# KaHIP/KaMinPar

Measured on NVIDIA H100. Metric: lp_edges_per_second, higher is better.
Workload: dtype int32

## Files before the change

kaminpar_b200/csrc/lp_device.cuh:

```cuda
#pragma once

#include <cstdint>
#include <cuda_runtime.h>

namespace kmp {

constexpr uint32_t kEmpty = 0xFFFFFFFFu;
constexpr unsigned kFull = 0xFFFFFFFFu;
constexpr int kLadderLevels = 16;

enum : uint32_t { SALT_SUBROUND = 1, SALT_TIE = 2, SALT_FAV = 3, SALT_COMMIT = 4 };

__host__ __device__ __forceinline__ uint32_t lowbias32(uint32_t x) {
  x ^= x >> 16;
  x *= 0x7FEB352Du;
  x ^= x >> 15;
  x *= 0x846CA68Bu;
  x ^= x >> 16;
  return x;
}
__host__ __device__ __forceinline__ uint32_t tie_hash(uint32_t base, uint32_t u, uint32_t c) {
  return lowbias32((u * 0x9E3779B1u) ^ (c * 0x85EBCA77u) ^ base);
}
__host__ __device__ __forceinline__ uint32_t bijective32(uint32_t x, uint32_t base) {
  x ^= base;
  x *= 0x9E3779B1u;
  x ^= x >> 15;
  x *= 0x85EBCA77u;
  x ^= x >> 13;
  x *= 0xC2B2AE3Du;
  x ^= x >> 16;
  return x;
}
__host__ __device__ __forceinline__ uint32_t subround_of(uint32_t u, uint32_t granule_log2,
                                                         uint32_t base, uint32_t S) {
  const uint32_t h = lowbias32((u >> granule_log2) ^ base);
  return static_cast<uint32_t>((static_cast<uint64_t>(h) * S) >> 32);
}
__device__ __forceinline__ uint32_t ladder_level(uint32_t prio) {
  const uint32_t z = static_cast<uint32_t>(__clz(static_cast<int>(prio)));
  return z < static_cast<uint32_t>(kLadderLevels - 1) ? z : static_cast<uint32_t>(kLadderLevels - 1);
}
__host__ __device__ __forceinline__ uint32_t degree_group(uint32_t d) {
  return d < 8 ? 0u : (d < 32 ? 1u : (d < 256 ? 2u : 3u));
}

inline uint64_t splitmix64(uint64_t x) {
  x += 0x9E3779B97F4A7C15ull;
  x = (x ^ (x >> 30)) * 0xBF58476D1CE4E5B9ull;
  x = (x ^ (x >> 27)) * 0x94D049BB133111EBull;
  return x ^ (x >> 31);
}
inline uint32_t sync_base(int seed, uint32_t call, uint32_t iter, uint32_t salt) {
  const uint64_t a = splitmix64((static_cast<uint64_t>(static_cast<uint32_t>(seed)) << 32) | call);
  const uint64_t b = splitmix64((static_cast<uint64_t>(iter) << 32) | salt);
  return static_cast<uint32_t>(splitmix64(a ^ b) >> 32);
}

struct Cand {
  int32_t gain;
  int32_t over;
  uint32_t hash;
  uint32_t key;
};
__device__ __forceinline__ Cand cand_none() { return Cand{-1, 0, kEmpty, kEmpty}; }

template <int MODE> __device__ __forceinline__ bool cand_better(const Cand &a, const Cand &b) {
  if (a.gain != b.gain) {
    return a.gain > b.gain;
  }
  if (MODE == 1 && a.over != b.over) {
    return a.over < b.over;
  }
  if (a.hash != b.hash) {
    return a.hash < b.hash;
  }
  return a.key < b.key;
}

template <int MODE> __device__ __forceinline__ Cand warp_argmax(unsigned mask, Cand c) {
  const int gmax = __reduce_max_sync(mask, c.gain);
  bool in = (c.gain == gmax) && (gmax > 0);
  int omin = 0;
  if (MODE == 1) {
    omin = __reduce_min_sync(mask, in ? c.over : INT32_MAX);
    in = in && (c.over == omin);
  }
  const unsigned hmin = __reduce_min_sync(mask, in ? c.hash : kEmpty);
  in = in && (c.hash == hmin);
  const unsigned kmin = __reduce_min_sync(mask, in ? c.key : kEmpty);
  Cand r;
  r.gain = gmax > 0 ? gmax : -1;
  r.over = omin;
  r.hash = hmin;
  r.key = kmin;
  return r;
}

constexpr uint32_t kStampBits = 6;
constexpr uint32_t kMaxStampSubrounds = 1u << kStampBits;
template <bool P64> struct LabG;
template <> struct LabG<false> {
  using word = uint32_t;
  static __host__ __device__ __forceinline__ uint32_t label(word w) { return w & 0x00FFFFFFu; }
  static __host__ __device__ __forceinline__ uint32_t stamp(word w) { return w >> 24; }
  static __host__ __device__ __forceinline__ word pack(uint32_t label, uint32_t stamp) { return label | (stamp << 24); }
};
template <> struct LabG<true> {
  using word = unsigned long long;
  static __host__ __device__ __forceinline__ uint32_t label(word w) { return static_cast<uint32_t>(w); }
  static __host__ __device__ __forceinline__ uint32_t stamp(word w) { return static_cast<uint32_t>(w >> 32); }
  static __host__ __device__ __forceinline__ word pack(uint32_t label, uint32_t stamp) {
    return static_cast<word>(label) | (static_cast<word>(stamp) << 32);
  }
};
__host__ __device__ __forceinline__ uint32_t make_stamp(uint32_t round, uint32_t subround) {
  return 1u + ((round & 1u) << kStampBits) + subround;
}
struct StampWindow {
  uint32_t start, len;
};
__host__ __device__ __forceinline__ StampWindow make_window(uint32_t round, uint32_t subround) {
  return StampWindow{(((round & 1u) ^ 1u) << kStampBits) + subround, (2u << kStampBits) - subround};
}
__device__ __forceinline__ bool stamp_hit(uint32_t stamp, const StampWindow &w) {
  return stamp != 0 && ((stamp - 1u - w.start) & ((2u << kStampBits) - 1u)) < w.len;
}

constexpr int kCounterNodesOffset = 16;
struct SweepArgs {
  const uint32_t *__restrict__ xadj;
  const uint32_t *__restrict__ adjncy;
  const int32_t *__restrict__ vwgt;
  const int32_t *__restrict__ adjwgt;
  const uint32_t *__restrict__ label;
  const void *__restrict__ labg;
  StampWindow window;
  bool pull;
  uint32_t *__restrict__ queue;
  const int32_t *__restrict__ weight;
  const int32_t *__restrict__ max_w;
  const int32_t *__restrict__ min_w;
  const uint32_t *__restrict__ communities;
  uint8_t *__restrict__ active;
  uint32_t *__restrict__ favored;
  int32_t max_cluster_weight;
  uint32_t num_labels;
  uint32_t max_num_neighbors;
  const uint32_t *__restrict__ list;
  uint32_t list_size;
  uint32_t base_tie, base_fav, base_commit;
  uint32_t *__restrict__ mv_u;
  uint32_t *__restrict__ mv_t;
  uint32_t *__restrict__ mover_count;
  bool accumulate;
  int32_t *__restrict__ incoming;
  int32_t *__restrict__ hist;
  unsigned long long *__restrict__ counters;
  uint32_t *__restrict__ sel_target;
  uint32_t *__restrict__ sel_favored;
};

template <int MODE>
__device__ __forceinline__ Cand eval_candidate_w(const SweepArgs &a, uint32_t u, uint32_t own, int32_t uw,
                                                 int32_t own_w, uint32_t key, int32_t rating, int32_t kw,
                                                 bool store_fav, Cand &fav) {
  Cand c = cand_none();
  fav = cand_none();
  if (rating <= 0) {
    return c;
  }
  if (MODE == 0) {
    bool feasible = (kw + uw <= a.max_cluster_weight) || (key == own);
    if (a.communities != nullptr) {
      feasible = feasible && (a.communities[key] == a.communities[own]);
    }
    if (feasible) {
      c.gain = rating;
      c.over = 0;
      c.hash = tie_hash(a.base_tie, u, key);
      c.key = key;
    }
    if (store_fav) {
      fav.gain = rating;
      fav.over = 0;
      fav.hash = tie_hash(a.base_fav, u, key);
      fav.key = key;
    }
  } else {
    const int32_t kmax = a.max_w[key];
    const int32_t over = kw - kmax;
    const int32_t init_over = own_w - a.max_w[own];
    const bool feasible = (kw + uw <= kmax) || (over < init_over) || (key == own);
    if (feasible) {
      c.gain = rating;
      c.over = over;
      c.hash = tie_hash(a.base_tie, u, key);
      c.key = key;
    }
  }
  return c;
}

template <int MODE>
__device__ __forceinline__ Cand eval_candidate(const SweepArgs &a, uint32_t u, uint32_t own, int32_t uw,
                                               int32_t own_w, uint32_t key, int32_t rating, bool store_fav,
                                               Cand &fav) {
  if (rating <= 0) {
    fav = cand_none();
    return cand_none();
  }
  return eval_candidate_w<MODE>(a, u, own, uw, own_w, key, rating, a.weight[key], store_fav, fav);
}

template <int MODE>
__device__ __forceinline__ bool finish_vertex(const SweepArgs &a, uint32_t u, uint32_t own, bool store_fav,
                                              const Cand &best, const Cand &fav, uint32_t &target_out) {
  const uint32_t target = best.gain > 0 ? best.key : own;
  target_out = target;
  if (a.sel_target != nullptr) {
    a.sel_target[u] = target;
    if (MODE == 0 && a.sel_favored != nullptr) {
      a.sel_favored[u] = store_fav ? (fav.gain > 0 ? fav.key : own) : kEmpty;
    }
    return false;
  }
  if (target != own) {
    return true;
  }
  if (MODE == 0 && store_fav) {
    a.favored[u] = fav.gain > 0 ? fav.key : own;
  }
  return false;
}

}
```

kaminpar_b200/csrc/lp_sweep.cuh:

```cuda
#pragma once

#include "lp_device.cuh"
#include "lp_sortnet.cuh"

namespace kmp {

template <int MODE>
__device__ __forceinline__ void emit_proposal(const SweepArgs &a, uint32_t idx, uint32_t u, uint32_t target,
                                              int32_t uw) {
  a.mv_u[idx] = u;
  a.mv_t[idx] = target;
  if (!a.accumulate) {
    return;
  }
  if (MODE == 0) {
    atomicAdd(&a.incoming[target], uw);
  } else {
    const uint32_t lvl = ladder_level(bijective32(u, a.base_commit));
    atomicAdd(&a.hist[target * kLadderLevels + lvl], uw);
  }
}

__device__ __forceinline__ void block_count_flush(const SweepArgs &a, unsigned long long edges,
                                                  unsigned long long nodes) {
  for (int o = 16; o > 0; o >>= 1) {
    edges += __shfl_xor_sync(kFull, edges, o);
    nodes += __shfl_xor_sync(kFull, nodes, o);
  }
  if ((threadIdx.x & 31) == 0 && nodes != 0) {
    atomicAdd(&a.counters[0], edges);
    atomicAdd(&a.counters[kCounterNodesOffset], nodes);
  }
}

template <bool P64>
__device__ __forceinline__ typename LabG<P64>::word load_labg(const SweepArgs &a, uint32_t v) {
  return static_cast<const typename LabG<P64>::word *>(a.labg)[v];
}

template <int R> struct ThreadRow {
  uint32_t u, beg, deg;
  uint32_t v[R > 0 ? R : 1];
};
template <int R> __device__ __forceinline__ void load_row(const SweepArgs &a, ThreadRow<R> &r) {
  r.beg = a.xadj[r.u];
  const uint32_t deg = a.xadj[r.u + 1] - r.beg;
  r.deg = deg > a.max_num_neighbors ? a.max_num_neighbors : deg;
#pragma unroll
  for (int j = 0; j < R; ++j) {
    r.v[j] = j < static_cast<int>(r.deg) ? a.adjncy[r.beg + j] : 0u;
  }
}

template <int MODE, bool EW, bool P64, int N, int R>
__device__ __forceinline__ bool sweep_thread_vertex(const SweepArgs &a, const ThreadRow<R> &r, bool flag,
                                                    unsigned long long &edges, unsigned long long &nodes,
                                                    uint32_t &target, int32_t &uw) {
  const uint32_t u = r.u;
  const uint32_t own = a.label[u];
  uw = a.vwgt != nullptr ? a.vwgt[u] : 1;
  const int32_t own_w = a.weight[own];
  uint32_t keys[N];
  int32_t ws[N];
  bool hit = false;
#pragma unroll
  for (int j = 0; j < N; ++j) {
    keys[j] = kEmpty;
    ws[j] = 0;
    if (j < static_cast<int>(r.deg)) {
      const uint32_t v = R > 0 ? r.v[j] : a.adjncy[r.beg + j];
      const typename LabG<P64>::word g = load_labg<P64>(a, v);
      hit = hit || stamp_hit(LabG<P64>::stamp(g), a.window);
      bool ok = true;
      if (MODE == 1 && a.communities != nullptr) {
        ok = a.communities[u] == a.communities[v];
      }
      if (ok) {
        keys[j] = LabG<P64>::label(g);
        ws[j] = EW ? a.adjwgt[r.beg + j] : 1;
      }
    }
  }
  if (!(flag || hit)) {
    return false;
  }
  edges += r.deg;
  nodes += 1;
  if (a.active != nullptr && flag) {
    a.active[u] = 0;
  }
  bool skip = false;
  if (MODE == 1) {
    const int32_t mn = a.min_w != nullptr ? a.min_w[own] : 0;
    skip = (own_w - uw) < mn;
  }
  const bool store_fav = (MODE == 0) && (uw == own_w) && (own_w <= a.max_cluster_weight / 2);
  Cand best = cand_none(), fav = cand_none();
  if (!skip) {
    sort_registers<N, EW>(keys, ws);
    bool lazy_done = false;
    if (MODE == 0) {
      Cand top = cand_none();
      int32_t run = 0;
#pragma unroll
      for (int j = 0; j < N; ++j) {
        run += EW ? ws[j] : 1;
        const bool last = (j == N - 1) || (keys[j + 1 < N ? j + 1 : j] != keys[j]);
        if (last) {
          const int32_t rating = run;
          run = 0;
          if (keys[j] != kEmpty && rating > 0) {
            if (rating >= top.gain) {
              const Cand x{rating, 0, tie_hash(a.base_tie, u, keys[j]), keys[j]};
              if (cand_better<0>(x, top)) {
                top = x;
              }
            }
            if (store_fav && rating >= fav.gain) {
              const Cand y{rating, 0, tie_hash(a.base_fav, u, keys[j]), keys[j]};
              if (cand_better<0>(y, fav)) {
                fav = y;
              }
            }
          }
        }
      }
      bool top_ok = true;
      if (top.gain > 0) {
        top_ok = (a.weight[top.key] + uw <= a.max_cluster_weight) || (top.key == own);
        if (a.communities != nullptr) {
          top_ok = top_ok && (a.communities[top.key] == a.communities[own]);
        }
      }
      if (top_ok) {
        best = top;
        lazy_done = true;
      }
    }
    if (!lazy_done) {
      int32_t run = 0;
#pragma unroll
      for (int j = 0; j < N; ++j) {
        run += EW ? ws[j] : 1;
        const bool last = (j == N - 1) || (keys[j + 1 < N ? j + 1 : j] != keys[j]);
        if (last) {
          const int32_t rating = run;
          run = 0;
          if (keys[j] != kEmpty) {
            Cand f;
            const Cand c = eval_candidate<MODE>(a, u, own, uw, own_w, keys[j], rating, MODE == 0 ? false : store_fav, f);
            if (cand_better<MODE>(c, best)) {
              best = c;
            }
          }
        }
      }
    }
  }
  return finish_vertex<MODE>(a, u, own, store_fav, best, fav, target);
}

template <int MODE>
__device__ __forceinline__ void emit_cta_iteration(const SweepArgs &a, bool proposes, uint32_t u, uint32_t target,
                                                   int32_t uw, uint32_t it, uint32_t (&s_cnt)[2][8],
                                                   uint32_t (&s_base)[2]) {
  const unsigned ballot = __ballot_sync(kFull, proposes);
  const int lane = threadIdx.x & 31;
  const int wib = threadIdx.x >> 5;
  const int par = it & 1;
  if (lane == 0) {
    s_cnt[par][wib] = static_cast<uint32_t>(__popc(ballot));
  }
  __syncthreads();
  if (threadIdx.x == 0) {
    uint32_t total = 0;
    for (int w = 0; w < 8; ++w) {
      total += s_cnt[par][w];
    }
    s_base[par] = total != 0 ? atomicAdd(a.mover_count, total) : 0u;
  }
  __syncthreads();
  if (proposes) {
    uint32_t idx = s_base[par] + __popc(ballot & ((1u << lane) - 1u));
    for (int w = 0; w < wib; ++w) {
      idx += s_cnt[par][w];
    }
    emit_proposal<MODE>(a, idx, u, target, uw);
  }
}

template <int MODE, bool EW, bool P64, int N> __global__ void __launch_bounds__(256) sweep_thread(const SweepArgs a) {
  __shared__ uint32_t s_cnt[2][8];
  __shared__ uint32_t s_base[2];
  unsigned long long edges = 0, nodes = 0;
  const uint32_t stride = gridDim.x * blockDim.x;
  const uint32_t bound = (a.list_size + 255u) & ~255u;
  uint32_t it = 0;
  for (uint32_t i = blockIdx.x * blockDim.x + threadIdx.x; i < bound; i += stride, ++it) {
    bool proposes = false;
    uint32_t target = 0;
    int32_t uw = 1;
    ThreadRow<0> r;
    r.u = 0;
    if (i < a.list_size) {
      r.u = a.list[i];
      const bool flag = a.active == nullptr || a.active[r.u] != 0;
      if (flag || a.pull) {
        load_row<0>(a, r);
        proposes = sweep_thread_vertex<MODE, EW, P64, N>(a, r, flag, edges, nodes, target, uw);
      }
    }
    emit_cta_iteration<MODE>(a, proposes, r.u, target, uw, it, s_cnt, s_base);
  }
  block_count_flush(a, edges, nodes);
}

__device__ __forceinline__ uint32_t pow2_ceil(uint32_t x) {
  return x <= 1 ? 1u : (1u << (32 - __clz(static_cast<int>(x - 1))));
}

__device__ __forceinline__ void table_add(uint32_t *keys, int32_t *vals, uint32_t mask, bool direct, uint32_t key,
                                          int32_t w) {
  uint32_t slot = direct ? key : (lowbias32(key) & mask);
  while (true) {
    const uint32_t prev = atomicCAS(&keys[slot], kEmpty, key);
    if (prev == kEmpty || prev == key) {
      atomicAdd(&vals[slot], w);
      return;
    }
    slot = (slot + 1) & mask;
  }
}

template <int T> struct TeamSync {
  static __device__ __forceinline__ void sync(int id) {
    if (T == 32) {
      __syncwarp();
    } else {
      asm volatile("bar.sync %0, %1;" ::"r"(id), "r"(T) : "memory");
    }
  }
  static __device__ __forceinline__ bool any(int id, bool p) {
    if (T == 32) {
      __syncwarp();
      return __any_sync(kFull, p);
    } else {
      int r;
      asm volatile(
          "{\n"
          ".reg .pred q, r;\n"
          "setp.ne.s32 q, %3, 0;\n"
          "bar.red.or.pred r, %1, %2, q;\n"
          "selp.s32 %0, 1, 0, r;\n"
          "}\n"
          : "=r"(r)
          : "r"(id), "r"(T), "r"(static_cast<int>(p))
          : "memory");
      return r != 0;
    }
  }
};

template <int MODE, int T>
__device__ __forceinline__ Cand team_argmax(int id, int tid, Cand c, Cand *s_red) {
  Cand r = warp_argmax<MODE>(kFull, c);
  if (T == 32) {
    return r;
  }
  TeamSync<T>::sync(id);
  if ((tid & 31) == 0) {
    s_red[tid >> 5] = r;
  }
  TeamSync<T>::sync(id);
  Cand x = cand_none();
  if ((tid & 31) < T / 32) {
    x = s_red[tid & 31];
  }
  return warp_argmax<MODE>(kFull, x);
}

template <bool V16> struct TeamVals;
template <> struct TeamVals<false> {
  using word = int32_t;
  static constexpr int kBytesPerSlot = 4;
  static __device__ __forceinline__ void add(word *v, uint32_t slot, int32_t w) { atomicAdd(&v[slot], w); }
  static __device__ __forceinline__ int32_t get(const word *v, uint32_t slot) { return v[slot]; }
  static __device__ __forceinline__ void clear(word *v, uint32_t slot) { v[slot] = 0; }
};
template <> struct TeamVals<true> {
  using word = uint32_t;
  static constexpr int kBytesPerSlot = 2;
  static __device__ __forceinline__ void add(word *v, uint32_t slot, int32_t w) {
    atomicAdd(&v[slot >> 1], static_cast<uint32_t>(w) << ((slot & 1u) * 16u));
  }
  static __device__ __forceinline__ int32_t get(const word *v, uint32_t slot) {
    return static_cast<int32_t>((v[slot >> 1] >> ((slot & 1u) * 16u)) & 0xFFFFu);
  }
  static __device__ __forceinline__ void clear(word *v, uint32_t slot) { reinterpret_cast<uint16_t *>(v)[slot] = 0; }
};

template <bool V16, bool EW>
__device__ __forceinline__ bool team_table_add(uint32_t *keys, typename TeamVals<V16>::word *vals, uint32_t mask,
                                               bool direct, uint32_t key, int32_t w, uint32_t &slot) {
  slot = direct ? key : (lowbias32(key) & mask);
  while (true) {
    const uint32_t prev = atomicCAS(&keys[slot], kEmpty, key);
    if (!EW && prev == kEmpty) {
      return true;
    }
    if (prev == kEmpty || prev == key) {
      TeamVals<V16>::add(vals, slot, w);
      return prev == kEmpty;
    }
    slot = (slot + 1) & mask;
  }
}
template <bool V16, bool EW>
__device__ __forceinline__ int32_t team_rating(const typename TeamVals<V16>::word *vals, uint32_t slot) {
  return TeamVals<V16>::get(vals, slot) + (EW ? 0 : 1);
}

template <int T> constexpr int team_ctas_per_sm() { return T == 32 ? 6 : T == 1024 ? 1 : 3; }

template <int MODE, bool EW, bool P64, int T, int SLOTS, int TEAMS, bool V16 = false>
__global__ void __launch_bounds__(T *TEAMS, team_ctas_per_sm<T>()) sweep_team(const SweepArgs a) {
  static_assert((SLOTS & (SLOTS - 1)) == 0, "table size must be a power of two");
  static_assert(SLOTS <= 65536, "claim lists hold 16-bit slot indices");
  static_assert(!(V16 && EW), "16-bit ratings need unit edge weights");
  using TV = TeamVals<V16>;
  constexpr int kListCap = SLOTS / 2;
  extern __shared__ __align__(16) unsigned char smem_raw[];
  __shared__ Cand s_red_all[TEAMS][T > 32 ? T / 32 : 1];
  __shared__ uint16_t s_list_all[TEAMS][kListCap];
  __shared__ uint32_t s_next[TEAMS], s_claims[TEAMS];
  __shared__ unsigned long long s_edges[TEAMS], s_nodes[TEAMS];
  const int team = threadIdx.x / T;
  const int tid = threadIdx.x % T;
  const int lane = threadIdx.x & 31;
  const int bar = 1 + team;
  uint32_t *keys = reinterpret_cast<uint32_t *>(smem_raw) + static_cast<size_t>(team) * SLOTS;
  typename TV::word *vals = reinterpret_cast<typename TV::word *>(
      smem_raw + sizeof(uint32_t) * SLOTS * TEAMS + static_cast<size_t>(team) * SLOTS * TV::kBytesPerSlot);
  Cand *s_red = s_red_all[team];
  uint16_t *list = s_list_all[team];
  for (int s = tid; s < SLOTS; s += T) {
    keys[s] = kEmpty;
    TV::clear(vals, s);
  }
  uint32_t next = 0;
  unsigned long long edges = 0, nodes = 0;
  if (tid == 0) {
    next = atomicAdd(a.queue, 1u);
    if (T > 32) {
      s_edges[team] = 0;
      s_nodes[team] = 0;
    }
  }
  TeamSync<T>::sync(bar);
  while (true) {
    uint32_t i;
    if (T == 32) {
      i = __shfl_sync(kFull, next, 0);
    } else {
      if (tid == 0) {
        s_next[team] = next;
        s_claims[team] = 0;
      }
      TeamSync<T>::sync(bar);
      i = s_next[team];
    }
    if (i >= a.list_size) {
      break;
    }
    if (tid == 0) {
      next = atomicAdd(a.queue, 1u);
    }
    const uint32_t u = a.list[i];
    const bool flag = a.active == nullptr || a.active[u] != 0;
    if (!flag && !a.pull) {
      TeamSync<T>::sync(bar);
      continue;
    }
    const uint32_t beg = a.xadj[u];
    uint32_t deg = a.xadj[u + 1] - beg;
    if (deg > a.max_num_neighbors) {
      deg = a.max_num_neighbors;
    }
    const uint32_t own = a.label[u];
    const int32_t uw = a.vwgt != nullptr ? a.vwgt[u] : 1;
    const int32_t own_w = a.weight[own];
    bool skip = false;
    if (MODE == 1) {
      const int32_t mn = a.min_w != nullptr ? a.min_w[own] : 0;
      skip = (own_w - uw) < mn;
    }
    const bool direct = a.num_labels <= static_cast<uint32_t>(SLOTS);
    bool hit = false;
    uint32_t claims = 0;
    constexpr int B = 4;
    for (uint32_t e0 = 0; e0 < deg; e0 += T * B) {
      uint32_t kb[B];
      int32_t wb[B];
      uint32_t vb[B];
#pragma unroll
      for (int j = 0; j < B; ++j) {
        const uint32_t e = e0 + j * T + tid;
        vb[j] = e < deg ? a.adjncy[beg + e] : kEmpty;
        wb[j] = (EW && e < deg) ? a.adjwgt[beg + e] : 1;
      }
#pragma unroll
      for (int j = 0; j < B; ++j) {
        kb[j] = kEmpty;
        if (vb[j] != kEmpty) {
          const typename LabG<P64>::word g = load_labg<P64>(a, vb[j]);
          hit = hit || stamp_hit(LabG<P64>::stamp(g), a.window);
          bool ok = !skip;
          if (MODE == 1 && a.communities != nullptr) {
            ok = ok && a.communities[u] == a.communities[vb[j]];
          }
          if (ok) {
            kb[j] = LabG<P64>::label(g);
          }
        }
      }
      uint32_t sl[B];
      unsigned claimed[B];
#pragma unroll
      for (int j = 0; j < B; ++j) {
        sl[j] = 0;
        claimed[j] = __ballot_sync(kFull, kb[j] != kEmpty && team_table_add<V16, EW>(keys, vals, SLOTS - 1, direct,
                                                                                     kb[j], wb[j], sl[j]));
      }
      uint32_t n = 0;
#pragma unroll
      for (int j = 0; j < B; ++j) {
        n += __popc(claimed[j]);
      }
      if (n != 0) {
        uint32_t base = claims;
        if (T == 32) {
          claims += n;
        } else {
          if (lane == 0) {
            base = atomicAdd(&s_claims[team], n);
          }
          base = __shfl_sync(kFull, base, 0);
        }
        const unsigned below = (1u << lane) - 1u;
#pragma unroll
        for (int j = 0; j < B; ++j) {
          if ((claimed[j] >> lane) & 1u) {
            list[base + __popc(claimed[j] & below)] = static_cast<uint16_t>(sl[j]);
          }
          base += __popc(claimed[j]);
        }
      }
    }
    const bool any_hit = TeamSync<T>::any(bar, hit);
    const bool act = flag || any_hit;
    const uint32_t nc = T == 32 ? claims : s_claims[team];
    const bool store_fav = (MODE == 0) && (uw == own_w) && (own_w <= a.max_cluster_weight / 2);
    Cand best = cand_none(), fav = cand_none();
    if (act) {
      Cand c = cand_none(), f = cand_none();
      if (MODE == 0) {
        for (uint32_t l = tid; l < nc; l += T) {
          const uint32_t s = list[l];
          const uint32_t k = keys[s];
          const int32_t r = team_rating<V16, EW>(vals, s);
          if (r >= c.gain) {
            Cand x{r, 0, tie_hash(a.base_tie, u, k), k};
            if (cand_better<0>(x, c)) {
              c = x;
            }
          }
          if (store_fav && r >= f.gain) {
            Cand y{r, 0, tie_hash(a.base_fav, u, k), k};
            if (cand_better<0>(y, f)) {
              f = y;
            }
          }
        }
        const Cand top = team_argmax<0, T>(bar, tid, c, s_red);
        if (store_fav) {
          fav = team_argmax<0, T>(bar, tid, f, s_red);
        }
        bool top_ok = true;
        if (top.gain > 0) {
          top_ok = (a.weight[top.key] + uw <= a.max_cluster_weight) || (top.key == own);
          if (a.communities != nullptr) {
            top_ok = top_ok && (a.communities[top.key] == a.communities[own]);
          }
        }
        if (top_ok) {
          best = top;
        } else {
          Cand cb = cand_none();
          for (uint32_t l0 = 0; l0 < nc; l0 += T * 4) {
            uint32_t kk[4];
            int32_t rr[4], ww[4];
#pragma unroll
            for (int j = 0; j < 4; ++j) {
              const uint32_t l = l0 + j * T + tid;
              const uint32_t s = l < nc ? list[l] : 0u;
              kk[j] = l < nc ? keys[s] : kEmpty;
              rr[j] = l < nc ? team_rating<V16, EW>(vals, s) : 0;
            }
#pragma unroll
            for (int j = 0; j < 4; ++j) {
              ww[j] = kk[j] != kEmpty ? a.weight[kk[j]] : 0;
            }
#pragma unroll
            for (int j = 0; j < 4; ++j) {
              if (kk[j] != kEmpty) {
                Cand ff;
                const Cand cc = eval_candidate_w<0>(a, u, own, uw, own_w, kk[j], rr[j], ww[j], false, ff);
                if (cand_better<0>(cc, cb)) {
                  cb = cc;
                }
              }
            }
          }
          best = team_argmax<0, T>(bar, tid, cb, s_red);
        }
      } else {
        for (uint32_t l = tid; l < nc; l += T) {
          const uint32_t s = list[l];
          const uint32_t k = keys[s];
          Cand ff;
          const Cand cc = eval_candidate_w<1>(a, u, own, uw, own_w, k, team_rating<V16, EW>(vals, s), a.weight[k], false, ff);
          if (cand_better<1>(cc, c)) {
            c = cc;
          }
        }
        best = team_argmax<1, T>(bar, tid, c, s_red);
      }
    }
    for (uint32_t l = tid; l < nc; l += T) {
      const uint32_t s = list[l];
      keys[s] = kEmpty;
      TV::clear(vals, s);
    }
    if (act && tid == 0) {
      if (T == 32) {
        edges += deg;
        nodes += 1;
      } else {
        s_edges[team] += deg;
        s_nodes[team] += 1;
      }
      if (a.active != nullptr && flag) {
        a.active[u] = 0;
      }
      uint32_t target;
      if (finish_vertex<MODE>(a, u, own, store_fav, best, fav, target)) {
        const uint32_t idx = atomicAdd(a.mover_count, 1u);
        emit_proposal<MODE>(a, idx, u, target, uw);
      }
    }
    TeamSync<T>::sync(bar);
  }
  if (T > 32 && tid == 0) {
    edges = s_edges[team];
    nodes = s_nodes[team];
  }
  if (tid == 0 && nodes != 0) {
    atomicAdd(&a.counters[0], edges);
    atomicAdd(&a.counters[kCounterNodesOffset], nodes);
  }
}

constexpr int kChunkEdges = 2048;
constexpr int kSliceEdges = 256;
constexpr int kSliceTableSlots = 512;
constexpr int kChunkThreads = 256;
constexpr uint32_t kBucketCap = 512;
constexpr uint32_t kBucketTargetFill = 256;
constexpr uint32_t kSelTableSlots = 1024;
constexpr int kSelWarps = 4;

struct HubOverflow {
  uint32_t bucket;
  uint32_t key;
  int32_t rating;
  uint32_t pad;
};

struct HubArgs {
  const uint32_t *__restrict__ item_entry;
  const uint32_t *__restrict__ item_chunk;
  const uint32_t *__restrict__ item_u;
  const uint32_t *__restrict__ item_beg;
  const uint32_t *__restrict__ item_deg;
  uint32_t num_items;
  const uint32_t *__restrict__ table_off;
  unsigned long long *__restrict__ g_tab;
  uint32_t *__restrict__ cursor;
  HubOverflow *__restrict__ ovf;
  uint32_t *__restrict__ ovf_count;
  uint32_t ovf_cap;
  uint32_t bucket_cap;
  uint32_t sel_limit;
  uint32_t stage_adjncy;
  const uint32_t *__restrict__ sel_entry;
  const uint32_t *__restrict__ sel_piece;
  uint32_t num_sel_items;
  const uint32_t *__restrict__ sel_begin;
  Cand *__restrict__ part_best;
  Cand *__restrict__ part_fav;
  uint32_t rank, world;
  uint32_t *__restrict__ queue;
  uint32_t *__restrict__ hit;
};

__host__ __device__ __forceinline__ uint32_t hub_buckets(uint32_t full_degree) {
  const uint32_t need = (full_degree + kBucketTargetFill - 1) / kBucketTargetFill;
  uint32_t p = 1;
  while (p < need) {
    p <<= 1;
  }
  return p;
}

__device__ __forceinline__ uint32_t smem_u32(const void *p) {
  return static_cast<uint32_t>(__cvta_generic_to_shared(p));
}
__device__ __forceinline__ void mbar_init(uint64_t *bar, uint32_t count) {
  asm volatile("mbarrier.init.shared::cta.b64 [%0], %1;" ::"r"(smem_u32(bar)), "r"(count) : "memory");
}
__device__ __forceinline__ void mbar_arrive_expect_tx(uint64_t *bar, uint32_t bytes) {
  asm volatile("mbarrier.arrive.expect_tx.shared::cta.b64 _, [%0], %1;" ::"r"(smem_u32(bar)), "r"(bytes) : "memory");
}
__device__ __forceinline__ void mbar_wait(uint64_t *bar, uint32_t parity) {
  asm volatile(
      "{\n"
      ".reg .pred p;\n"
      "WAIT_LOOP:\n"
      "mbarrier.try_wait.parity.shared::cta.b64 p, [%0], %1;\n"
      "@p bra DONE;\n"
      "bra WAIT_LOOP;\n"
      "DONE:\n"
      "}\n" ::"r"(smem_u32(bar)),
      "r"(parity)
      : "memory");
}
__device__ __forceinline__ void tma_load_1d(void *dst_smem, const void *src_gmem, uint32_t bytes, uint64_t *bar) {
  asm volatile("cp.async.bulk.shared::cluster.global.mbarrier::complete_tx::bytes [%0], [%1], %2, [%3];" ::"r"(
                   smem_u32(dst_smem)),
               "l"(src_gmem), "r"(bytes), "r"(smem_u32(bar))
               : "memory");
}

struct HubItem {
  uint32_t valid;
  uint32_t u;
  uint32_t entry;
  uint32_t full_deg;
  uint32_t gbeg, gend;
  uint32_t a0;
  uint32_t staged;
};

__device__ __forceinline__ void mbar_arrive(uint64_t *bar) {
  asm volatile("mbarrier.arrive.shared::cta.b64 _, [%0];" ::"r"(smem_u32(bar)) : "memory");
}

constexpr int kHubStages = 2;
constexpr int kHubConsumerWarps = kChunkThreads / 32;
constexpr int kHubThreads = kChunkThreads + 32;
constexpr int kHubScatterSmem = kHubConsumerWarps * kSliceTableSlots * 8;

template <int MODE, bool EW, bool P64>
__global__ void __launch_bounds__(kHubThreads, 4) sweep_hub_scatter(const SweepArgs a, const HubArgs hb, uint32_t m_total) {
  extern __shared__ __align__(16) unsigned char smem_raw[];
  constexpr int kAllSlots = kHubConsumerWarps * kSliceTableSlots;
  uint32_t *all_keys = reinterpret_cast<uint32_t *>(smem_raw);
  int32_t *all_vals = reinterpret_cast<int32_t *>(smem_raw + sizeof(uint32_t) * kAllSlots);
  __shared__ __align__(16) uint32_t s_adj[kHubStages][kChunkEdges + 8];
  __shared__ __align__(8) uint64_t s_full[kHubStages];
  __shared__ __align__(8) uint64_t s_empty[kHubStages];
  __shared__ HubItem s_item[kHubStages];
  const int lane = threadIdx.x & 31;
  const int wib = threadIdx.x >> 5;
  if (threadIdx.x == 0) {
    for (int s = 0; s < kHubStages; ++s) {
      mbar_init(&s_full[s], 1);
      mbar_init(&s_empty[s], kHubConsumerWarps);
    }
    asm volatile("fence.mbarrier_init.release.cluster;" ::: "memory");
  }
  for (int s = threadIdx.x; s < kAllSlots; s += kHubThreads) {
    all_keys[s] = kEmpty;
    all_vals[s] = 0;
  }
  __syncthreads();

  if (wib == kHubConsumerWarps) {
    if (lane == 0) {
      for (uint32_t k = 0;; ++k) {
        const int stage = static_cast<int>(k % kHubStages);
        const uint32_t round = k / kHubStages;
        mbar_wait(&s_empty[stage], (round & 1u) ^ 1u);
        const uint32_t it = atomicAdd(hb.queue, 1u);
        HubItem d{};
        d.valid = 0;
        if (it >= hb.num_items) {
          d.valid = 2;
          s_item[stage] = d;
          mbar_arrive(&s_full[stage]);
          break;
        }
        const uint32_t entry = hb.item_entry[it];
        const uint32_t u = hb.item_u[it];
        const uint32_t beg0 = hb.item_beg[it];
        const uint32_t full_deg = hb.item_deg[it];
        const uint32_t chunk = hb.item_chunk[it];
        if (entry % hb.world == hb.rank && (a.active == nullptr || a.pull || a.active[u] != 0)) {
          uint32_t deg = full_deg;
          if (deg > a.max_num_neighbors) {
            deg = a.max_num_neighbors;
          }
          const uint32_t cbeg = chunk * kChunkEdges;
          bool ok = cbeg < deg;
          if (ok && MODE == 1) {
            const uint32_t own = a.label[u];
            const int32_t uw = a.vwgt != nullptr ? a.vwgt[u] : 1;
            const int32_t mn = a.min_w != nullptr ? a.min_w[own] : 0;
            ok = !((a.weight[own] - uw) < mn);
          }
          if (ok) {
            const uint32_t cend = (cbeg + kChunkEdges < deg) ? cbeg + kChunkEdges : deg;
            d.valid = 1;
            d.u = u;
            d.entry = entry;
            d.full_deg = full_deg;
            d.gbeg = beg0 + cbeg;
            d.gend = beg0 + cend;
            d.a0 = d.gbeg & ~3u;
            d.staged = 0;
            if (hb.stage_adjncy) {
              uint32_t a1 = (d.gend + 3u) & ~3u;
              const uint32_t m4 = m_total & ~3u;
              if (a1 > m4) {
                a1 = m4;
              }
              d.staged = a1 > d.a0 ? a1 - d.a0 : 0;
            }
          }
        }
        s_item[stage] = d;
        if (d.valid && d.staged > 0) {
          asm volatile("fence.proxy.async.shared::cta;" ::: "memory");
          mbar_arrive_expect_tx(&s_full[stage], d.staged * 4);
          tma_load_1d(&s_adj[stage][0], a.adjncy + d.a0, d.staged * 4, &s_full[stage]);
        } else {
          mbar_arrive(&s_full[stage]);
        }
      }
    }
    return;
  }

  uint32_t *keys = all_keys + wib * kSliceTableSlots;
  int32_t *vals = all_vals + wib * kSliceTableSlots;
  for (uint32_t k = 0;; ++k) {
    const int stage = static_cast<int>(k % kHubStages);
    const uint32_t round = k / kHubStages;
    mbar_wait(&s_full[stage], round & 1u);
    const HubItem d = s_item[stage];
    if (d.valid == 2) {
      break;
    }
    const uint32_t wbeg = d.gbeg + wib * kSliceEdges;
    const bool mine = d.valid && wbeg < d.gend;
    if (mine) {
      const uint32_t wend = wbeg + kSliceEdges < d.gend ? wbeg + kSliceEdges : d.gend;
      const uint32_t staged_end = d.a0 + d.staged;
      bool hit = false;
      for (uint32_t e0 = wbeg; e0 < wend; e0 += 128) {
        uint32_t k4[4];
        int32_t w4[4];
#pragma unroll
        for (int j = 0; j < 4; ++j) {
          const uint32_t e = e0 + j * 32 + lane;
          k4[j] = kEmpty;
          w4[j] = 0;
          if (e < wend) {
            const uint32_t v = e < staged_end ? s_adj[stage][e - d.a0] : a.adjncy[e];
            bool ok = true;
            if (MODE == 1 && a.communities != nullptr) {
              ok = a.communities[d.u] == a.communities[v];
            }
            const typename LabG<P64>::word g = load_labg<P64>(a, v);
            hit = hit || stamp_hit(LabG<P64>::stamp(g), a.window);
            if (ok) {
              k4[j] = LabG<P64>::label(g);
              w4[j] = EW ? a.adjwgt[e] : 1;
            }
          }
        }
#pragma unroll
        for (int j = 0; j < 4; ++j) {
          if (k4[j] != kEmpty) {
            table_add(keys, vals, kSliceTableSlots - 1, false, k4[j], w4[j]);
          }
        }
      }
      if (a.pull && __any_sync(kFull, hit) && lane == 0) {
        atomicOr(&hb.hit[d.entry], 1u);
      }
    }
    __syncwarp();
    if (lane == 0) {
      mbar_arrive(&s_empty[stage]);
    }
    if (mine) {
      const uint32_t pmask = hub_buckets(d.full_deg) - 1;
      const uint32_t bucket0 = hb.table_off[d.entry];
      constexpr int B = 4;
      for (uint32_t s0 = lane; s0 < kSliceTableSlots; s0 += 32 * B) {
        uint32_t kk[B], bb[B], pos[B];
        int32_t rr[B];
#pragma unroll
        for (int j = 0; j < B; ++j) {
          const uint32_t s = s0 + j * 32;
          kk[j] = keys[s];
          rr[j] = vals[s];
          if (kk[j] != kEmpty) {
            keys[s] = kEmpty;
            vals[s] = 0;
          }
        }
#pragma unroll
        for (int j = 0; j < B; ++j) {
          bb[j] = bucket0 + (lowbias32(kk[j]) & pmask);
          pos[j] = kk[j] != kEmpty ? atomicAdd(&hb.cursor[bb[j]], 1u) : 0u;
        }
#pragma unroll
        for (int j = 0; j < B; ++j) {
          if (kk[j] != kEmpty) {
            if (pos[j] < hb.bucket_cap) {
              hb.g_tab[static_cast<size_t>(bb[j]) * kBucketCap + pos[j]] =
                  (static_cast<unsigned long long>(kk[j]) << 32) | static_cast<uint32_t>(rr[j]);
            } else {
              const uint32_t o = atomicAdd(hb.ovf_count, 1u);
              if (o < hb.ovf_cap) {
                hb.ovf[o] = HubOverflow{bb[j], kk[j], rr[j], 0u};
              }
            }
          }
        }
      }
      __syncwarp();
    }
  }
}

template <int MODE> __global__ void __launch_bounds__(kSelWarps * 32) sweep_hub_select(const SweepArgs a, const HubArgs hb) {
  __shared__ uint32_t s_keys[kSelWarps][kSelTableSlots];
  __shared__ int32_t s_vals[kSelWarps][kSelTableSlots];
  __shared__ uint32_t s_claims_all[kSelWarps];
  const int lane = threadIdx.x & 31;
  const int wib = threadIdx.x >> 5;
  uint32_t *keys = s_keys[wib];
  int32_t *vals = s_vals[wib];
  uint32_t *s_claims = &s_claims_all[wib];
  for (uint32_t s = lane; s < kSelTableSlots; s += 32) {
    keys[s] = kEmpty;
    vals[s] = 0;
  }
  if (lane == 0) {
// ... 246 lines not shown
```

Baseline: 41.13 billion.

## Split warp into half-warps to process two low-degree vertices concurrently

The warp-per-vertex sweep path now grabs two vertices per queue fetch. When both have small degree, each half-warp rates one vertex, using its own half of the shared hash table and a new half-warp argmax reduction. Otherwise the two vertices are processed one after the other by the full warp. Edge and node counters are kept in spare lanes' registers instead of separate accumulators. The aim is to cut idle lanes on low-degree vertices, at the cost of halved table capacity per vertex, extra reduction passes, and more complex control flow.

```diff
diff --git a/kaminpar_b200/csrc/lp_device.cuh b/kaminpar_b200/csrc/lp_device.cuh
--- a/kaminpar_b200/csrc/lp_device.cuh
+++ b/kaminpar_b200/csrc/lp_device.cuh
@@ -89,6 +89,36 @@
   const unsigned hmin = __reduce_min_sync(mask, in ? c.hash : kEmpty);
   in = in && (c.hash == hmin);
   const unsigned kmin = __reduce_min_sync(mask, in ? c.key : kEmpty);
+  Cand r;
+  r.gain = gmax > 0 ? gmax : -1;
+  r.over = omin;
+  r.hash = hmin;
+  r.key = kmin;
+  return r;
+}
+
+template <int MODE> __device__ __forceinline__ Cand half_warp_argmax(Cand c) {
+  const bool hi = (threadIdx.x & 16u) != 0;
+  const auto max2 = [hi](int v) {
+    const int lo_r = __reduce_max_sync(kFull, hi ? INT32_MIN : v);
+    const int hi_r = __reduce_max_sync(kFull, hi ? v : INT32_MIN);
+    return hi ? hi_r : lo_r;
+  };
+  const auto min2 = [hi](auto v, decltype(v) neutral) {
+    const auto lo_r = __reduce_min_sync(kFull, hi ? neutral : v);
+    const auto hi_r = __reduce_min_sync(kFull, hi ? v : neutral);
+    return hi ? hi_r : lo_r;
+  };
+  const int gmax = max2(c.gain);
+  bool in = (c.gain == gmax) && (gmax > 0);
+  int omin = 0;
+  if (MODE == 1) {
+    omin = min2(in ? c.over : INT32_MAX, INT32_MAX);
+    in = in && (c.over == omin);
+  }
+  const unsigned hmin = min2(in ? c.hash : kEmpty, kEmpty);
+  in = in && (c.hash == hmin);
+  const unsigned kmin = min2(in ? c.key : kEmpty, kEmpty);
   Cand r;
   r.gain = gmax > 0 ? gmax : -1;
   r.over = omin;
diff --git a/kaminpar_b200/csrc/lp_sweep.cuh b/kaminpar_b200/csrc/lp_sweep.cuh
--- a/kaminpar_b200/csrc/lp_sweep.cuh
+++ b/kaminpar_b200/csrc/lp_sweep.cuh
@@ -1,4 +1,6 @@
 #pragma once
+
+#include <type_traits>
 
 #include "lp_device.cuh"
 #include "lp_sortnet.cuh"
@@ -347,226 +349,435 @@
     keys[s] = kEmpty;
     TV::clear(vals, s);
   }
-  uint32_t next = 0;
-  unsigned long long edges = 0, nodes = 0;
-  if (tid == 0) {
-    next = atomicAdd(a.queue, 1u);
-    if (T > 32) {
+  if constexpr (T == 32) {
+    constexpr int kNodeLane = 1, kEdgeLane = 2, kPairLane = 3;
+    uint32_t next = 0;
+    if (lane == 0) {
+      next = atomicAdd(a.queue, 2u);
+    }
+    __syncwarp();
+    while (true) {
+      const uint32_t i = __shfl_sync(kFull, next, 0);
+      if (i >= a.list_size) {
+        break;
+      }
+      if (lane == 0) {
+        next = atomicAdd(a.queue, 2u);
+      }
+      uint32_t u, beg, deg;
+      bool flag;
+      const auto load_header = [&](uint32_t j) {
+        const bool valid = j < a.list_size;
+        u = a.list[valid ? j : j - 1];
+        flag = valid && (a.active == nullptr || a.active[u] != 0);
+        beg = a.xadj[u];
+        deg = a.xadj[u + 1] - beg;
+        if (deg > a.max_num_neighbors) {
+          deg = a.max_num_neighbors;
+        }
+        if (!flag && !(valid && a.pull)) {
+          deg = 0;
+        }
+      };
+      const auto rate = [&](auto half_tag) {
+        constexpr bool HALF = decltype(half_tag)::value;
+        constexpr int width = HALF ? 16 : 32;
+        constexpr unsigned kBits = HALF ? 0xFFFFu : kFull;
+        const int me = HALF ? (lane & 15) : lane;
+        const int hofs = HALF ? (lane & 16) : 0;
+        constexpr uint32_t tslots = HALF ? SLOTS / 2 : SLOTS;
+        uint32_t *tkeys = keys + hofs * (SLOTS / 32);
+        typename TV::word *tvals = vals + hofs * (SLOTS / 32) * TV::kBytesPerSlot / static_cast<int>(sizeof(typename TV::word));
+        uint16_t *tlist = list + hofs * (kListCap / 32);
+        const auto team_max = [](Cand c) { return HALF ? half_warp_argmax<MODE>(c) : warp_argmax<MODE>(kFull, c); };
+        const uint32_t own = a.label[u];
+        const int32_t uw = a.vwgt != nullptr ? a.vwgt[u] : 1;
+        const int32_t own_w = a.weight[own];
+        if (me == 0 && a.active != nullptr && flag) {
+          a.active[u] = 0;
+        }
+        bool skip = false;
+        if (MODE == 1) {
+          const int32_t mn = a.min_w != nullptr ? a.min_w[own] : 0;
+          skip = (own_w - uw) < mn;
+        }
+        const bool direct = a.num_labels <= tslots;
+        bool hit = false;
+        uint32_t claims = 0;
+        constexpr int B = 4;
+        for (uint32_t e0 = 0; __any_sync(kFull, e0 < deg); e0 += width * B) {
+          uint32_t kb[B];
+          int32_t wb[B];
+          uint32_t vb[B];
+#pragma unroll
+          for (int j = 0; j < B; ++j) {
+            const uint32_t e = e0 + j * width + me;
+            vb[j] = e < deg ? a.adjncy[beg + e] : kEmpty;
+            wb[j] = (EW && e < deg) ? a.adjwgt[beg + e] : 1;
+          }
+#pragma unroll
+          for (int j = 0; j < B; ++j) {
+            kb[j] = kEmpty;
+            if (vb[j] != kEmpty) {
+              const typename LabG<P64>::word g = load_labg<P64>(a, vb[j]);
+              hit = hit || stamp_hit(LabG<P64>::stamp(g), a.window);
+              bool ok = !skip;
+              if (MODE == 1 && a.communities != nullptr) {
+                ok = ok && a.communities[u] == a.communities[vb[j]];
+              }
+              if (ok) {
+                kb[j] = LabG<P64>::label(g);
+              }
+            }
+          }
+          const unsigned below = (1u << me) - 1u;
+#pragma unroll
+          for (int j = 0; j < B; ++j) {
+            uint32_t sl = 0;
+            const unsigned claimed = __ballot_sync(kFull, kb[j] != kEmpty && team_table_add<V16, EW>(
+                                                                                  tkeys, tvals, tslots - 1, direct,
+                                                                                  kb[j], wb[j], sl)) >>
+                                         hofs &
+                                     kBits;
+            if ((claimed >> me) & 1u) {
+              tlist[claims + __popc(claimed & below)] = static_cast<uint16_t>(sl);
+            }
+            claims += __popc(claimed);
+          }
+        }
+        __syncwarp();
+        const bool any_hit = ((__ballot_sync(kFull, hit) >> hofs) & kBits) != 0;
+        const bool act = flag || any_hit;
+        if (act) {
+          next += me == kNodeLane ? 1u : me == kEdgeLane ? deg : 0u;
+        }
+        const uint32_t nc = claims;
+        const bool store_fav = (MODE == 0) && (uw == own_w) && (own_w <= a.max_cluster_weight / 2);
+        const auto either = [](bool p) { return HALF ? __any_sync(kFull, p) : p; };
+        const uint32_t ns = act ? nc : 0u;
+        Cand best = cand_none(), fav = cand_none();
+        if (either(act)) {
+          Cand c = cand_none(), f = cand_none();
+          if (MODE == 0) {
+            for (uint32_t l = me; l < ns; l += width) {
+              const uint32_t s = tlist[l];
+              const uint32_t k = tkeys[s];
+              const int32_t r = team_rating<V16, EW>(tvals, s);
+              if (r >= c.gain) {
+                Cand x{r, 0, tie_hash(a.base_tie, u, k), k};
+                if (cand_better<0>(x, c)) {
+                  c = x;
+                }
+              }
+              if (store_fav && r >= f.gain) {
+                Cand y{r, 0, tie_hash(a.base_fav, u, k), k};
+                if (cand_better<0>(y, f)) {
+                  f = y;
+                }
+              }
+            }
+            const Cand top = team_max(c);
+            if (either(store_fav)) {
+              fav = team_max(f);
+            }
+            bool top_ok = true;
+            if (top.gain > 0) {
+              top_ok = (a.weight[top.key] + uw <= a.max_cluster_weight) || (top.key == own);
+              if (a.communities != nullptr) {
+                top_ok = top_ok && (a.communities[top.key] == a.communities[own]);
+              }
+            }
+            best = top;
+            if (either(!top_ok)) {
+              const uint32_t nb = top_ok ? 0u : ns;
+              Cand cb = cand_none();
+              constexpr int PB = 2;
+              for (uint32_t l0 = 0; l0 < nb; l0 += width * PB) {
+                uint32_t kk[PB];
+                int32_t rr[PB], ww[PB];
+#pragma unroll
+                for (int j = 0; j < PB; ++j) {
+                  const uint32_t l = l0 + j * width + me;
+                  const uint32_t s = l < nb ? tlist[l] : 0u;
+                  kk[j] = l < nb ? tkeys[s] : kEmpty;
+                  rr[j] = l < nb ? team_rating<V16, EW>(tvals, s) : 0;
+                }
+#pragma unroll
+                for (int j = 0; j < PB; ++j) {
+                  ww[j] = kk[j] != kEmpty ? a.weight[kk[j]] : 0;
+                }
+#pragma unroll
+                for (int j = 0; j < PB; ++j) {
+                  if (kk[j] != kEmpty) {
+                    Cand ff;
+                    const Cand cc = eval_candidate_w<0>(a, u, own, uw, own_w, kk[j], rr[j], ww[j], false, ff);
+                    if (cand_better<0>(cc, cb)) {
+                      cb = cc;
+                    }
+                  }
+                }
+              }
+              const Cand all = team_max(cb);
+              if (!top_ok) {
+                best = all;
+              }
+            }
+          } else {
+            for (uint32_t l = me; l < ns; l += width) {
+              const uint32_t s = tlist[l];
+              const uint32_t k = tkeys[s];
+              Cand ff;
+              const Cand cc =
+                  eval_candidate_w<1>(a, u, own, uw, own_w, k, team_rating<V16, EW>(tvals, s), a.weight[k], false, ff);
+              if (cand_better<1>(cc, c)) {
+                c = cc;
+              }
+            }
+            best = team_max(c);
+          }
+        }
+        for (uint32_t l = me; l < nc; l += width) {
+          const uint32_t s = tlist[l];
+          tkeys[s] = kEmpty;
+          TV::clear(tvals, s);
+        }
+        if (act && me == 0) {
+          uint32_t target;
+          if (finish_vertex<MODE>(a, u, own, store_fav, best, fav, target)) {
+            const uint32_t idx = atomicAdd(a.mover_count, 1u);
+            emit_proposal<MODE>(a, idx, u, target, uw);
+          }
+        }
+        __syncwarp();
+      };
+      {
+        load_header(i + (lane >> 4));
+        if (__reduce_max_sync(kFull, deg) < static_cast<uint32_t>(SLOTS / 4)) {
+          rate(std::true_type{});
+        } else {
+          if (lane == kPairLane) {
+            next = i;
+          }
+#pragma unroll 1
+          for (uint32_t p = 0; p < 2; ++p) {
+            load_header(__shfl_sync(kFull, next, kPairLane) + p);
+            rate(std::false_type{});
+          }
+        }
+      }
+    }
+    const unsigned long long nodes = __shfl_sync(kFull, next, kNodeLane) + __shfl_sync(kFull, next, 16 + kNodeLane);
+    const unsigned long long edges =
+        static_cast<unsigned long long>(__shfl_sync(kFull, next, kEdgeLane)) + __shfl_sync(kFull, next, 16 + kEdgeLane);
+    if (lane == 0 && nodes != 0) {
+      atomicAdd(&a.counters[0], edges);
+      atomicAdd(&a.counters[kCounterNodesOffset], nodes);
+    }
+  } else {
+    uint32_t next = 0;
+    unsigned long long edges = 0, nodes = 0;
+    if (tid == 0) {
+      next = atomicAdd(a.queue, 1u);
       s_edges[team] = 0;
       s_nodes[team] = 0;
     }
-  }
-  TeamSync<T>::sync(bar);
-  while (true) {
-    uint32_t i;
-    if (T == 32) {
-      i = __shfl_sync(kFull, next, 0);
-    } else {
+    TeamSync<T>::sync(bar);
+    while (true) {
       if (tid == 0) {
         s_next[team] = next;
         s_claims[team] = 0;
       }
       TeamSync<T>::sync(bar);
-      i = s_next[team];
-    }
-    if (i >= a.list_size) {
-      break;
-    }
-    if (tid == 0) {
-      next = atomicAdd(a.queue, 1u);
-    }
-    const uint32_t u = a.list[i];
-    const bool flag = a.active == nullptr || a.active[u] != 0;
-    if (!flag && !a.pull) {
-      TeamSync<T>::sync(bar);
-      continue;
-    }
-    const uint32_t beg = a.xadj[u];
-    uint32_t deg = a.xadj[u + 1] - beg;
-    if (deg > a.max_num_neighbors) {
-      deg = a.max_num_neighbors;
-    }
-    const uint32_t own = a.label[u];
-    const int32_t uw = a.vwgt != nullptr ? a.vwgt[u] : 1;
-    const int32_t own_w = a.weight[own];
-    bool skip = false;
-    if (MODE == 1) {
-      const int32_t mn = a.min_w != nullptr ? a.min_w[own] : 0;
-      skip = (own_w - uw) < mn;
-    }
-    const bool direct = a.num_labels <= static_cast<uint32_t>(SLOTS);
-    bool hit = false;
-    uint32_t claims = 0;
-    constexpr int B = 4;
-    for (uint32_t e0 = 0; e0 < deg; e0 += T * B) {
-      uint32_t kb[B];
-      int32_t wb[B];
-      uint32_t vb[B];
-#pragma unroll
-      for (int j = 0; j < B; ++j) {
-        const uint32_t e = e0 + j * T + tid;
-        vb[j] = e < deg ? a.adjncy[beg + e] : kEmpty;
-        wb[j] = (EW && e < deg) ? a.adjwgt[beg + e] : 1;
-      }
-#pragma unroll
-      for (int j = 0; j < B; ++j) {
-        kb[j] = kEmpty;
-        if (vb[j] != kEmpty) {
-          const typename LabG<P64>::word g = load_labg<P64>(a, vb[j]);
-          hit = hit || stamp_hit(LabG<P64>::stamp(g), a.window);
-          bool ok = !skip;
-          if (MODE == 1 && a.communities != nullptr) {
-            ok = ok && a.communities[u] == a.communities[vb[j]];
-          }
-          if (ok) {
-            kb[j] = LabG<P64>::label(g);
-          }
-        }
-      }
-      uint32_t sl[B];
-      unsigned claimed[B];
-#pragma unroll
-      for (int j = 0; j < B; ++j) {
-        sl[j] = 0;
-        claimed[j] = __ballot_sync(kFull, kb[j] != kEmpty && team_table_add<V16, EW>(keys, vals, SLOTS - 1, direct,
-                                                                                     kb[j], wb[j], sl[j]));
-      }
-      uint32_t n = 0;
-#pragma unroll
-      for (int j = 0; j < B; ++j) {
-        n += __popc(claimed[j]);
-      }
-      if (n != 0) {
-        uint32_t base = claims;
-        if (T == 32) {
-          claims += n;
-        } else {
+      const uint32_t i = s_next[team];
+      if (i >= a.list_size) {
+        break;
+      }
+      if (tid == 0) {
+        next = atomicAdd(a.queue, 1u);
+      }
+      const uint32_t u = a.list[i];
+      const bool flag = a.active == nullptr || a.active[u] != 0;
+      if (!flag && !a.pull) {
+        TeamSync<T>::sync(bar);
+        continue;
+      }
+      const uint32_t beg = a.xadj[u];
+      uint32_t deg = a.xadj[u + 1] - beg;
+      if (deg > a.max_num_neighbors) {
+        deg = a.max_num_neighbors;
+      }
+      const uint32_t own = a.label[u];
+      const int32_t uw = a.vwgt != nullptr ? a.vwgt[u] : 1;
+      const int32_t own_w = a.weight[own];
+      bool skip = false;
+      if (MODE == 1) {
+        const int32_t mn = a.min_w != nullptr ? a.min_w[own] : 0;
+        skip = (own_w - uw) < mn;
+      }
+      const bool direct = a.num_labels <= static_cast<uint32_t>(SLOTS);
+      bool hit = false;
+      constexpr int B = 4;
+      for (uint32_t e0 = 0; e0 < deg; e0 += T * B) {
+        uint32_t kb[B];
+        int32_t wb[B];
+        uint32_t vb[B];
+#pragma unroll
+        for (int j = 0; j < B; ++j) {
+          const uint32_t e = e0 + j * T + tid;
+          vb[j] = e < deg ? a.adjncy[beg + e] : kEmpty;
+          wb[j] = (EW && e < deg) ? a.adjwgt[beg + e] : 1;
+        }
+#pragma unroll
+        for (int j = 0; j < B; ++j) {
+          kb[j] = kEmpty;
+          if (vb[j] != kEmpty) {
+            const typename LabG<P64>::word g = load_labg<P64>(a, vb[j]);
+            hit = hit || stamp_hit(LabG<P64>::stamp(g), a.window);
+            bool ok = !skip;
+            if (MODE == 1 && a.communities != nullptr) {
+              ok = ok && a.communities[u] == a.communities[vb[j]];
+            }
+            if (ok) {
+              kb[j] = LabG<P64>::label(g);
+            }
+          }
+        }
+        uint32_t sl[B];
+        unsigned claimed[B];
+#pragma unroll
+        for (int j = 0; j < B; ++j) {
+          sl[j] = 0;
+          claimed[j] = __ballot_sync(kFull, kb[j] != kEmpty && team_table_add<V16, EW>(keys, vals, SLOTS - 1, direct,
+                                                                                       kb[j], wb[j], sl[j]));
+        }
+        uint32_t n = 0;
+#pragma unroll
+        for (int j = 0; j < B; ++j) {
+          n += __popc(claimed[j]);
+        }
+        if (n != 0) {
+          uint32_t base = 0;
           if (lane == 0) {
             base = atomicAdd(&s_claims[team], n);
           }
           base = __shfl_sync(kFull, base, 0);
-        }
-        const unsigned below = (1u << lane) - 1u;
-#pragma unroll
-        for (int j = 0; j < B; ++j) {
-          if ((claimed[j] >> lane) & 1u) {
-            list[base + __popc(claimed[j] & below)] = static_cast<uint16_t>(sl[j]);
-          }
-          base += __popc(claimed[j]);
-        }
-      }
-    }
-    const bool any_hit = TeamSync<T>::any(bar, hit);
-    const bool act = flag || any_hit;
-    const uint32_t nc = T == 32 ? claims : s_claims[team];
-    const bool store_fav = (MODE == 0) && (uw == own_w) && (own_w <= a.max_cluster_weight / 2);
-    Cand best = cand_none(), fav = cand_none();
-    if (act) {
-      Cand c = cand_none(), f = cand_none();
-      if (MODE == 0) {
-        for (uint32_t l = tid; l < nc; l += T) {
-          const uint32_t s = list[l];
-          const uint32_t k = keys[s];
-          const int32_t r = team_rating<V16, EW>(vals, s);
-          if (r >= c.gain) {
-            Cand x{r, 0, tie_hash(a.base_tie, u, k), k};
-            if (cand_better<0>(x, c)) {
-              c = x;
-            }
-          }
-          if (store_fav && r >= f.gain) {
-            Cand y{r, 0, tie_hash(a.base_fav, u, k), k};
-            if (cand_better<0>(y, f)) {
-              f = y;
-            }
-          }
-        }
-        const Cand top = team_argmax<0, T>(bar, tid, c, s_red);
-        if (store_fav) {
-          fav = team_argmax<0, T>(bar, tid, f, s_red);
-        }
-        bool top_ok = true;
-        if (top.gain > 0) {
-          top_ok = (a.weight[top.key] + uw <= a.max_cluster_weight) || (top.key == own);
-          if (a.communities != nullptr) {
-            top_ok = top_ok && (a.communities[top.key] == a.communities[own]);
-          }
-        }
-        if (top_ok) {
-          best = top;
+          const unsigned below = (1u << lane) - 1u;
+#pragma unroll
+          for (int j = 0; j < B; ++j) {
+            if ((claimed[j] >> lane) & 1u) {
+              list[base + __popc(claimed[j] & below)] = static_cast<uint16_t>(sl[j]);
+            }
+            base += __popc(claimed[j]);
+          }
+        }
+      }
+      const bool any_hit = TeamSync<T>::any(bar, hit);
+      const bool act = flag || any_hit;
+      const uint32_t nc = s_claims[team];
+      const bool store_fav = (MODE == 0) && (uw == own_w) && (own_w <= a.max_cluster_weight / 2);
+      Cand best = cand_none(), fav = cand_none();
+      if (act) {
+        Cand c = cand_none(), f = cand_none();
+        if (MODE == 0) {
+          for (uint32_t l = tid; l < nc; l += T) {
+            const uint32_t s = list[l];
+            const uint32_t k = keys[s];
+            const int32_t r = team_rating<V16, EW>(vals, s);
+            if (r >= c.gain) {
+              Cand x{r, 0, tie_hash(a.base_tie, u, k), k};
+              if (cand_better<0>(x, c)) {
+                c = x;
+              }
+            }
+            if (store_fav && r >= f.gain) {
+              Cand y{r, 0, tie_hash(a.base_fav, u, k), k};
+              if (cand_better<0>(y, f)) {
+                f = y;
+              }
+            }
+          }
+          const Cand top = team_argmax<0, T>(bar, tid, c, s_red);
+          if (store_fav) {
+            fav = team_argmax<0, T>(bar, tid, f, s_red);
+          }
+          bool top_ok = true;
+          if (top.gain > 0) {
+            top_ok = (a.weight[top.key] + uw <= a.max_cluster_weight) || (top.key == own);
+            if (a.communities != nullptr) {
+              top_ok = top_ok && (a.communities[top.key] == a.communities[own]);
+            }
+          }
+          if (top_ok) {
+            best = top;
+          } else {
+            Cand cb = cand_none();
+            for (uint32_t l0 = 0; l0 < nc; l0 += T * 4) {
+              uint32_t kk[4];
+              int32_t rr[4], ww[4];
+#pragma unroll
+              for (int j = 0; j < 4; ++j) {
+                const uint32_t l = l0 + j * T + tid;
+                const uint32_t s = l < nc ? list[l] : 0u;
+                kk[j] = l < nc ? keys[s] : kEmpty;
+                rr[j] = l < nc ? team_rating<V16, EW>(vals, s) : 0;
+              }
+#pragma unroll
+              for (int j = 0; j < 4; ++j) {
+                ww[j] = kk[j] != kEmpty ? a.weight[kk[j]] : 0;
+              }
+#pragma unroll
+              for (int j = 0; j < 4; ++j) {
+                if (kk[j] != kEmpty) {
+                  Cand ff;
+                  const Cand cc = eval_candidate_w<0>(a, u, own, uw, own_w, kk[j], rr[j], ww[j], false, ff);
+                  if (cand_better<0>(cc, cb)) {
+                    cb = cc;
+                  }
+                }
+              }
+            }
+            best = team_argmax<0, T>(bar, tid, cb, s_red);
+          }
         } else {
-          Cand cb = cand_none();
-          for (uint32_t l0 = 0; l0 < nc; l0 += T * 4) {
-            uint32_t kk[4];
-            int32_t rr[4], ww[4];
-#pragma unroll
-            for (int j = 0; j < 4; ++j) {
-              const uint32_t l = l0 + j * T + tid;
-              const uint32_t s = l < nc ? list[l] : 0u;
-              kk[j] = l < nc ? keys[s] : kEmpty;
-              rr[j] = l < nc ? team_rating<V16, EW>(vals, s) : 0;
-            }
-#pragma unroll
-            for (int j = 0; j < 4; ++j) {
-              ww[j] = kk[j] != kEmpty ? a.weight[kk[j]] : 0;
-            }
-#pragma unroll
-            for (int j = 0; j < 4; ++j) {
-              if (kk[j] != kEmpty) {
-                Cand ff;
-                const Cand cc = eval_candidate_w<0>(a, u, own, uw, own_w, kk[j], rr[j], ww[j], false, ff);
-                if (cand_better<0>(cc, cb)) {
-                  cb = cc;
-                }
-              }
-            }
-          }
-          best = team_argmax<0, T>(bar, tid, cb, s_red);
-        }
-      } else {
-        for (uint32_t l = tid; l < nc; l += T) {
-          const uint32_t s = list[l];
-          const uint32_t k = keys[s];
-          Cand ff;
-          const Cand cc = eval_candidate_w<1>(a, u, own, uw, own_w, k, team_rating<V16, EW>(vals, s), a.weight[k], false, ff);
-          if (cand_better<1>(cc, c)) {
-            c = cc;
-          }
-        }
-        best = team_argmax<1, T>(bar, tid, c, s_red);
-      }
-    }
-    for (uint32_t l = tid; l < nc; l += T) {
-      const uint32_t s = list[l];
-      keys[s] = kEmpty;
-      TV::clear(vals, s);
-    }
-    if (act && tid == 0) {
-      if (T == 32) {
-        edges += deg;
-        nodes += 1;
-      } else {
+          for (uint32_t l = tid; l < nc; l += T) {
+            const uint32_t s = list[l];
+            const uint32_t k = keys[s];
+            Cand ff;
+            const Cand cc = eval_candidate_w<1>(a, u, own, uw, own_w, k, team_rating<V16, EW>(vals, s), a.weight[k], false, ff);
+            if (cand_better<1>(cc, c)) {
+              c = cc;
+            }
+          }
+          best = team_argmax<1, T>(bar, tid, c, s_red);
+        }
+      }
+      for (uint32_t l = tid; l < nc; l += T) {
+        const uint32_t s = list[l];
+        keys[s] = kEmpty;
+        TV::clear(vals, s);
+      }
+      if (act && tid == 0) {
         s_edges[team] += deg;
         s_nodes[team] += 1;
-      }
-      if (a.active != nullptr && flag) {
-        a.active[u] = 0;
-      }
-      uint32_t target;
-      if (finish_vertex<MODE>(a, u, own, store_fav, best, fav, target)) {
-        const uint32_t idx = atomicAdd(a.mover_count, 1u);
-        emit_proposal<MODE>(a, idx, u, target, uw);
-      }
-    }
-    TeamSync<T>::sync(bar);
-  }
-  if (T > 32 && tid == 0) {
-    edges = s_edges[team];
-    nodes = s_nodes[team];
-  }
-  if (tid == 0 && nodes != 0) {
-    atomicAdd(&a.counters[0], edges);
-    atomicAdd(&a.counters[kCounterNodesOffset], nodes);
+        if (a.active != nullptr && flag) {
+          a.active[u] = 0;
+        }
+        uint32_t target;
+        if (finish_vertex<MODE>(a, u, own, store_fav, best, fav, target)) {
+          const uint32_t idx = atomicAdd(a.mover_count, 1u);
+          emit_proposal<MODE>(a, idx, u, target, uw);
+        }
+      }
+      TeamSync<T>::sync(bar);
+    }
+    if (tid == 0) {
+      edges = s_edges[team];
+      nodes = s_nodes[team];
+    }
+    if (tid == 0 && nodes != 0) {
+      atomicAdd(&a.counters[0], edges);
+      atomicAdd(&a.counters[kCounterNodesOffset], nodes);
+    }
   }
 }
 
```

New measurement: 41.96 billion, median of 6. +2.0%, better.
